# Stanford-NavLab/NavLab-DPE-SDR

Hardware: AMD Instinct MI355X
Metric: manifold gridpoints x SVs correlated/sec (higher is better)
Workload: dtype f32

## Files before the change

### navlab-dpe-sdr_amd/csrc/dpe_bcs.hip

```cpp
#include <type_traits>

#include "dpe_common.h"
#include "dpe_prep.h"
#include "dpe_chm_dev.h"

namespace dpe {

constexpr int kSub = 256;
constexpr int kNMomMax = 6;
typedef float f2 __attribute__((ext_vector_type(2)));

__device__ __forceinline__ f2 cmul(f2 a, f2 b)
{
    f2 t, r;
    asm("v_pk_mul_f32 %0, %1, %2 op_sel_hi:[0,1]" : "=v"(t) : "v"(a), "v"(b));
    asm("v_pk_fma_f32 %0, %1, %2, %3 op_sel:[1,1,0] op_sel_hi:[1,0,1] neg_lo:[1,0,0]" : "=v"(r) : "v"(a), "v"(b), "v"(t));
    return r;
}

__device__ __forceinline__ f2 wipe_seed(float f)
{
    f2 w = f2{__builtin_amdgcn_cosf(f), -__builtin_amdgcn_sinf(f)};
    asm volatile("s_nop 1" : "+v"(w));
    return w;
// ... 35 lines not shown
        const int n4 = S >> 2;
        for (int n = gtid; n < n4; n += gsz) {
            const int4 v = x4[n];
            sI += (short)(v.x & 0xFFFF) + (short)(v.y & 0xFFFF) + (short)(v.z & 0xFFFF) + (short)(v.w & 0xFFFF);
            sQ += (v.x >> 16) + (v.y >> 16) + (v.z >> 16) + (v.w >> 16);
        }
        for (int n = (n4 << 2) + gtid; n < S; n += gsz) {
            const int v = x[n];
            sI += (short)(v & 0xFFFF);
            sQ += v >> 16;
        }
    } else {
        for (int n = gtid; n < S; n += gsz) {
            const int v = x[n];
            sI += (short)(v & 0xFFFF);
            sQ += v >> 16;
        }
    }
    long long tI = sI, tQ = sQ;
#pragma unroll
    for (int off = 32; off > 0; off >>= 1) {
        tI += __shfl_xor(tI, off, 64);
        tQ += __shfl_xor(tQ, off, 64);
    }
    __shared__ long long sW[4][2];
    if ((threadIdx.x & 63) == 0) { sW[threadIdx.x >> 6][0] = tI; sW[threadIdx.x >> 6][1] = tQ; }
    __syncthreads();
    if (threadIdx.x < 2) {
        long long *o = sums + ((size_t)w * kSumSlots + blockIdx.x) * 2;
        o[threadIdx.x] = sW[0][threadIdx.x] + sW[1][threadIdx.x] + sW[2][threadIdx.x] + sW[3][threadIdx.x];
    }
}

__global__ __launch_bounds__(256) void bcs_sum_kernel(const int16_t *__restrict__ iq, long long winStride, int S,
                                                      long long *__restrict__ sums, uint4 *__restrict__ upDst,
                                                      const uint4 *__restrict__ upSrc, int upN16)
{
    const int nThreads = gridDim.x * gridDim.y * 256;
    for (int i = (blockIdx.y * gridDim.x + blockIdx.x) * 256 + threadIdx.x; i < upN16; i += nThreads) upDst[i] = upSrc[i];
    sum_body(iq, winStride, S, sums);
}

struct BcsParamBlock {
    BcsChanDev c[DPE_MAX_CHAN];
    const int *guard;
};
__device__ __forceinline__ bool rerun_not_wanted(const BcsParamBlock &pb)
{
    return pb.guard != nullptr && (__hip_atomic_load(pb.guard, __ATOMIC_RELAXED, __HIP_MEMORY_SCOPE_AGENT) & 8) == 0;
}

__device__ __forceinline__ void window_mean(const long long *__restrict__ sums, int w, int nSumBlk, int S, float &mRe, float &mIm)
{
    const int lane = threadIdx.x & 63;
    long long tI = 0, tQ = 0;
    if (lane < nSumBlk) {
        const longlong2 v = *reinterpret_cast<const longlong2 *>(sums + ((size_t)w * kSumSlots + lane) * 2);
        tI = v.x; tQ = v.y;
    }
#pragma unroll
    for (int off = 32; off > 0; off >>= 1) {
        tI += __shfl_xor(tI, off, 64);
        tQ += __shfl_xor(tQ, off, 64);
    }
    mRe = (float)((double)tI / (double)(float)S);
    mIm = (float)((double)tQ / (double)(float)S);
}

template <int LH, int kNMom, bool TABLE, bool FUSE, bool CO = false>
__global__ __launch_bounds__(256) void bcs_bank_kernel(BcsParamBlock pb, int inl, const int16_t *__restrict__ iq, long long winStride, int S,
                                                       int K, int nSub, int tilesPerBlock, int nBlk, int vecOK, int nSumBlk, int lagShift,
                                                       const BcsChanDev *__restrict__ chan,
                                                       const long long *__restrict__ sums,
                                                       const int8_t *__restrict__ chipTable,
                                                       const double *__restrict__ tT,
                                                       float2 *__restrict__ part, float2 *__restrict__ mom,
                                                       float2 *__restrict__ momRep, long long *__restrict__ sumSlots, ChmKArgs co)
{
    constexpr int NL = 2 * LH + 1;
    constexpr int NREP = kSub + 2 * LH;
    constexpr int NRR = 4 + 2 * LH;
    __shared__ float sChips[2048];
    __shared__ __align__(16) float sRep[4][NREP + 4];
    __shared__ float2 sAcc[4][NL];
    if (rerun_not_wanted(pb)) return;

    int blkX = blockIdx.x;
    if constexpr (CO) {
        static_assert(FUSE && !TABLE, "the co-block rides in the single-window form");
        if (blkX == 0) {
            if (blockIdx.y == 0 && blockIdx.z == 0) chm_k2(co);
            else if (blockIdx.y == 1 && blockIdx.z == 0) chm_k3(co);
            return;
        }
        blkX -= 1;
    }
    const int blk = blkX, k = blockIdx.y, w = blockIdx.z;
    const int tid = threadIdx.x, wave = tid >> 6, lane = tid & 63;
    (void)pb;
    const BcsChanDev ch = params_ptr(chan, inl)[w * K + k];
    for (int i = tid; i < 2048; i += 256) sChips[i] = (float)chipTable[(ch.prn - 1) * 1024 + (i >= kLCA ? i - kLCA : i) % kLCA];
    const bool fastIdx = (double)NREP * ch.codeStep < 1000.0;
    float mRe = 0.f, mIm = 0.f;
    if (!FUSE) window_mean(sums, w, nSumBlk, S, mRe, mIm);
    int sumI = 0, sumQ = 0;
    __shared__ int sSum[4][2];
    const int16_t *x = iq + (size_t)w * winStride * 2;
    float xp[4];
#pragma unroll
    for (int i = 0; i < 4; ++i) xp[i] = (float)(4 * lane + i) - 127.5f;
    __syncthreads();

    for (int side = 0; side < 2; ++side) {
        f2 acc[NL];
#pragma unroll
        for (int j = 0; j < NL; ++j) acc[j] = f2{0.f, 0.f};

        for (int t = 0; t < tilesPerBlock; ++t) {
            const int sub = (blk * tilesPerBlock + t) * 4 + wave;
            const int sub0 = sub * kSub;
            const int lo = sub0 - LH - lagShift, hi = sub0 + kSub - 1 + LH - lagShift;
            bool active = sub < nSub;
            if (active) {
                if (!ch.hasFlip) active = (side == 0);
                else if (lo >= 0 && hi < S) active = (side == 0) ? (lo < ch.idxNext) : (hi >= ch.idxNext);
            }
            const int n0 = sub0 + 4 * lane;
            float re[4], im[4];
            const bool countRaw = FUSE && k == 0 && side == 0 && sub < nSub;
            if (active || countRaw) {
                int rawv[4];
                if (vecOK && n0 + 3 < S) {
                    const int4 v = *reinterpret_cast<const int4 *>(x + 2 * (size_t)n0);
                    rawv[0] = v.x; rawv[1] = v.y; rawv[2] = v.z; rawv[3] = v.w;
                } else {
#pragma unroll
                    for (int i = 0; i < 4; ++i) rawv[i] = (n0 + i < S) ? *reinterpret_cast<const int *>(x + 2 * (size_t)(n0 + i)) : 0;
                }
#pragma unroll
                for (int i = 0; i < 4; ++i) {
                    re[i] = (float)(short)(rawv[i] & 0xFFFF);
                    im[i] = (float)(rawv[i] >> 16);
                    if (countRaw) { sumI += (short)(rawv[i] & 0xFFFF); sumQ += rawv[i] >> 16; }
                }
            }
            if (active) {
                if (fastIdx && lo >= 0 && hi < S) {
                    const int ci0 = (int)floor(code_phase<TABLE>(ch, tT, lo));
                    const int shift = (ci0 % kLCA) - ci0;
                    const bool straddle = ch.hasFlip && lo < ch.idxNext && hi >= ch.idxNext;
                    for (int e = lane; e < NREP; e += 64) {
                        const int m = lo + e;
                        const int ci = (int)floor(code_phase<TABLE>(ch, tT, m)) + shift;
                        float r = sChips[ci];
                        if (straddle) r = ((m >= ch.idxNext) == (side == 1)) ? r : 0.f;
                        sRep[wave][e] = r;
                    }
                } else {
                    for (int e = lane; e < NREP; e += 64) {
                        int m = lo + e;
                        if (m < 0) m += S; else if (m >= S) m -= S;
                        const double cph = code_phase<TABLE>(ch, tT, m);
                        const int ci = ((int)floor(cph)) % kLCA;
                        const int sd = ch.hasFlip ? (m >= ch.idxNext) : 0;
                        sRep[wave][e] = (sd == side) ? sChips[ci] : 0.f;
                    }
                }
            }
            f2 M[kNMom], Mq[FUSE ? kNMom : 1];
#pragma unroll
            for (int p = 0; p < kNMom; ++p) M[p] = f2{0.f, 0.f};
#pragma unroll
            for (int p = 0; p < (FUSE ? kNMom : 1); ++p) Mq[p] = f2{0.f, 0.f};
            if (active) {
                double ph = carr_phase<TABLE>(ch, tT, n0 < S ? n0 : S - 1);
                ph -= floor(ph);
                const float f = (float)ph;
                f2 wv = wipe_seed(f);
                const f2 meanv = f2{mRe, mIm}, rotv = f2{ch.rotRe, ch.rotIm};
                float rr[NRR];
#pragma unroll
                for (int q = 0; q < NRR / 4; ++q) {
                    const float4 v = *reinterpret_cast<const float4 *>(&sRep[wave][4 * lane + 4 * q]);
                    rr[4 * q] = v.x; rr[4 * q + 1] = v.y; rr[4 * q + 2] = v.z; rr[4 * q + 3] = v.w;
                }
#pragma unroll
                for (int i = 0; i < 4; ++i) {
                    const f2 wrot = wv;
                    wv = table_fix<TABLE>(wrot, ch, tT, n0, i, S);
                    const f2 bb = cmul(f2{re[i], im[i]}, wv);
#pragma unroll
                    for (int j = 0; j < NL; ++j) {
                        const float r = rr[i + 2 * LH - j];
                        acc[j] = __builtin_elementwise_fma(bb, f2{r, r}, acc[j]);
                    }
                    const float r0 = (n0 + i < S) ? rr[i + LH] : 0.f;
                    if (FUSE) {
                        f2 cp = bb * r0, cq = wv * r0;
#pragma unroll
                        for (int p = 0; p < kNMom; ++p) {
                            M[p] += cp; Mq[p] += cq;
                            cp *= xp[i]; cq *= xp[i];
                        }
                    } else {
                        f2 cp = (bb - cmul(meanv, wv)) * r0;
#pragma unroll
                        for (int p = 0; p < kNMom; ++p) {
                            M[p] += cp;
                            cp *= xp[i];
                        }
                    }
                    wv = cmul(wrot, rotv);
                }
            }
            if (sub < nSub && lagShift == 0) {
                const size_t mo = ((((size_t)w * K + k) * 2 + side) * nSub + sub) * kNMom;
                float2 *o = mom + mo;
                if (active) {
                    float mm[2 * kNMom];
#pragma unroll
                    for (int p = 0; p < kNMom; ++p) { mm[2 * p] = M[p].x; mm[2 * p + 1] = M[p].y; }
                    dpp_sum_lane63(mm);
                    if (lane == 63) {
#pragma unroll
                        for (int p = 0; p < kNMom; ++p) o[p] = make_float2(mm[2 * p], mm[2 * p + 1]);
                    }
                    if (FUSE) {
#pragma unroll
                        for (int p = 0; p < kNMom; ++p) { mm[2 * p] = Mq[p].x; mm[2 * p + 1] = Mq[p].y; }
                        dpp_sum_lane63(mm);
                        if (lane == 63) {
#pragma unroll
                            for (int p = 0; p < kNMom; ++p) momRep[mo + p] = make_float2(mm[2 * p], mm[2 * p + 1]);
                        }
                    }
                } else if (lane < kNMom) {
                    o[lane] = make_float2(0.f, 0.f);
                    if (FUSE) momRep[mo + lane] = make_float2(0.f, 0.f);
                }
            }
        }
        {
            float aa[2 * NL];
#pragma unroll
            for (int j = 0; j < NL; ++j) { aa[2 * j] = acc[j].x; aa[2 * j + 1] = acc[j].y; }
            dpp_sum_lane63(aa);
            if (lane == 63) {
#pragma unroll
                for (int j = 0; j < NL; ++j) sAcc[wave][j] = make_float2(aa[2 * j], aa[2 * j + 1]);
            }
        }
        if (FUSE && k == 0 && side == 0) {
#pragma unroll
            for (int off = 32; off > 0; off >>= 1) {
                sumI += __shfl_xor(sumI, off, 64);
                sumQ += __shfl_xor(sumQ, off, 64);
            }
            if (lane == 0) { sSum[wave][0] = sumI; sSum[wave][1] = sumQ; }
        }
        __syncthreads();
        if (FUSE && k == 0 && side == 0 && tid < 2)
            sumSlots[((size_t)w * kSumSlots + blk) * 2 + tid] =
                (long long)sSum[0][tid] + (long long)sSum[1][tid] + (long long)sSum[2][tid] + (long long)sSum[3][tid];
        for (int j = tid; j < NL; j += 256) {
            float2 s = sAcc[0][j];
            s.x += sAcc[1][j].x; s.y += sAcc[1][j].y;
            s.x += sAcc[2][j].x; s.y += sAcc[2][j].y;
            s.x += sAcc[3][j].x; s.y += sAcc[3][j].y;
            part[((((size_t)w * K + k) * nBlk + blk) * 2 + side) * NL + j] = s;
        }
        __syncthreads();
    }
}

constexpr int kB16Blocks = 4;
template <int LH, int kNMom, bool TABLE>
__global__ __launch_bounds__(256, (LH <= 4 && !TABLE) ? kB16Blocks : 3) void bcs_bank16_kernel(BcsParamBlock pb, int inl, const int16_t *__restrict__ iq, long long winStride,
                                                         int S, int K, int nW, int nSub, int tilesPerBlock, int nBlk, int vecOK, int nSumBlk,
                                                         const BcsChanDev *__restrict__ chan,
                                                         const long long *__restrict__ sums,
                                                         const int8_t *__restrict__ chipTable,
                                                         const double *__restrict__ tT,
                                                         float2 *__restrict__ part, float2 *__restrict__ mom)
{
    constexpr int NL = 2 * LH + 1;
    constexpr int kPass = 1024;
    constexpr int NREP = kPass + 2 * LH;
    constexpr int NRR = 16 + 2 * LH;
    static_assert((8 + 2 * LH) % 4 == 0 && LH <= 8, "a segment's replica window is read as float4s");
    __shared__ float sChips[2048];
#ifdef DPE_B16_PAD
    constexpr int kRepLen = ((NREP + 8 + 15) / 16) * 20;
#define DPE_PAD16(e) ((e) + 4 * ((e) >> 4))
#else
    constexpr int kRepLen = NREP + 8;
#define DPE_PAD16(e) (e)
#endif
    __shared__ __align__(16) float sRep[4][kRepLen];
    __shared__ float2 sAcc[4][NL];

    const int slot = blockIdx.x >> 3, k = slot % K, tg = (slot / K) * 8 + (blockIdx.x & 7);
    if (tg >= nBlk * nW) return;
    const int w = tg / nBlk, blk = tg - w * nBlk;
    const int tid = threadIdx.x, wave = tid >> 6, lane = tid & 63;
    (void)pb;
    const BcsChanDev ch = params_ptr(chan, inl)[w * K + k];
    for (int i = tid; i < 2048; i += 256) sChips[i] = (float)chipTable[(ch.prn - 1) * 1024 + (i >= kLCA ? i - kLCA : i) % kLCA];
    const bool fastIdx = (double)NREP * ch.codeStep < 1000.0;
    float mRe, mIm;
    window_mean(sums, w, nSumBlk, S, mRe, mIm);
    const f2 meanv = f2{mRe, mIm}, rotv = f2{ch.rotRe, ch.rotIm};
    const int16_t *x = iq + (size_t)w * winStride * 2;
    const int padLane = DPE_PAD16(lane);
    (void)padLane;
    const float xbase = (float)(16 * (lane & 15)) - 127.5f;
    __syncthreads();

    for (int side = 0; side < 2; ++side) {
        f2 acc[NL];
#pragma unroll
        for (int j = 0; j < NL; ++j) acc[j] = f2{0.f, 0.f};
        bool anyActive = false;

        for (int t = 0; t < tilesPerBlock; ++t) {
            const int pass = (blk * tilesPerBlock + t) * 4 + wave;
            const int c0 = pass * kPass;
            const int lo = c0 - LH, hi = c0 + kPass - 1 + LH;
            bool active = c0 < S;
            if (active) {
                if (!ch.hasFlip) active = (side == 0);
                else if (lo >= 0 && hi < S) active = (side == 0) ? (lo < ch.idxNext) : (hi >= ch.idxNext);
            }
            anyActive |= active;
            const int n0 = c0 + 16 * lane;
            if (active) {
                if (fastIdx && lo >= 0 && hi < S) {
                    const int ci0 = (int)code_phase<TABLE>(ch, tT, lo);
                    const int shift = (ci0 % kLCA) - ci0;
                    const bool straddle = ch.hasFlip && lo < ch.idxNext && hi >= ch.idxNext;
                    if (!straddle) {
                        static_assert(NREP >= 1024 && NREP < 1024 + 64, "sixteen full rounds of 64 entries and a partial one");
                        if constexpr (TABLE) {
                            for (int e = lane; e < NREP; e += 64) sRep[wave][DPE_PAD16(e)] = sChips[(int)code_phase<TABLE>(ch, tT, lo + e) + shift];
                        } else {
#pragma unroll
                        for (int e0 = 0; e0 < 1024; e0 += 512) {
                            float v[8];
#pragma unroll
                            for (int j = 0; j < 8; ++j) v[j] = sChips[(int)code_phase<TABLE>(ch, tT, lo + e0 + 64 * j + lane) + shift];
#pragma unroll
                            for (int j = 0; j < 8; ++j) sRep[wave][DPE_PAD16(e0 + 64 * j) + padLane] = v[j];
                        }
                        if (1024 + lane < NREP) sRep[wave][DPE_PAD16(1024) + padLane] = sChips[(int)code_phase<TABLE>(ch, tT, lo + 1024 + lane) + shift];
                        }
                    } else {
                        for (int e = lane; e < NREP; e += 64) {
                            const int m = lo + e;
                            const float r = sChips[(int)code_phase<TABLE>(ch, tT, m) + shift];
                            sRep[wave][DPE_PAD16(e)] = ((m >= ch.idxNext) == (side == 1)) ? r : 0.f;
                        }
                    }
                } else {
                    for (int e = lane; e < NREP; e += 64) {
                        int m = lo + e;
                        if (m < 0) m += S; else if (m >= S) m -= S;
                        const double cph = code_phase<TABLE>(ch, tT, m);
                        const int ci = ((int)floor(cph)) % kLCA;
                        const int sd = ch.hasFlip ? (m >= ch.idxNext) : 0;
                        sRep[wave][DPE_PAD16(e)] = (sd == side) ? sChips[ci] : 0.f;
                    }
                }
            }
            f2 M[kNMom];
#pragma unroll
            for (int p = 0; p < kNMom; ++p) M[p] = f2{0.f, 0.f};
            auto segments = [&](auto allInTag) {
                constexpr bool kAllIn = decltype(allInTag)::value;
#pragma unroll 1
                for (int seg = 0; seg < 2; ++seg) {
                    const int ns = n0 + 8 * seg;
                    int raw[8];
                    if (vecOK && (kAllIn || ns + 7 < S)) {
#pragma unroll
                        for (int q = 0; q < 2; ++q) {
                            const int4 v = *reinterpret_cast<const int4 *>(x + 2 * (size_t)(ns + 4 * q));
                            raw[4 * q] = v.x; raw[4 * q + 1] = v.y; raw[4 * q + 2] = v.z; raw[4 * q + 3] = v.w;
                        }
                    } else {
#pragma unroll
                        for (int i = 0; i < 8; ++i) raw[i] = (ns + i < S) ? *reinterpret_cast<const int *>(x + 2 * (size_t)(ns + i)) : 0;
                    }
                    float rr[8 + 2 * LH];
#pragma unroll
                    for (int q = 0; q < (8 + 2 * LH) / 4; ++q) {
                        const float4 v = *reinterpret_cast<const float4 *>(&sRep[wave][DPE_PAD16(16 * lane + 8 * seg + 4 * q)]);
                        rr[4 * q] = v.x; rr[4 * q + 1] = v.y; rr[4 * q + 2] = v.z; rr[4 * q + 3] = v.w;
                    }
                    double ph = carr_phase<TABLE>(ch, tT, (kAllIn || ns < S) ? ns : S - 1);
                    ph -= floor(ph);
                    f2 wv = wipe_seed((float)ph);
                    const bool inside = kAllIn || ns + 7 < S;
                    f2 m[kNMom];
#pragma unroll
                    for (int p = 0; p < kNMom; ++p) m[p] = f2{0.f, 0.f};
#pragma unroll
                    for (int i = 0; i < 8; ++i) {
                        const f2 rawv = f2{(float)(short)(raw[i] & 0xFFFF), (float)(raw[i] >> 16)};
                        const f2 wrot = wv;
                        wv = table_fix<TABLE>(wrot, ch, tT, ns, i, S);
                        const f2 bb = cmul(rawv, wv);
#pragma unroll
                        for (int j = 0; j < NL; ++j) {
                            const float r = rr[i + 2 * LH - j];
                            acc[j] = __builtin_elementwise_fma(bb, f2{r, r}, acc[j]);
                        }
                        const float r0 = (inside || ns + i < S) ? rr[i + LH] : 0.f;
                        const f2 cp = (bb - cmul(meanv, wv)) * r0;
                        const float d = (float)i - 3.5f;
                        float dp = 1.f;
                        m[0] += cp;
#pragma unroll
                        for (int p = 1; p < kNMom; ++p) {
                            dp *= d;
                            m[p] = __builtin_elementwise_fma(cp, f2{dp, dp}, m[p]);
                        }
                        wv = cmul(wrot, rotv);
                    }
                    const float xc = xbase + (float)(8 * seg) + 3.5f;
                    float xpow[kNMom];
                    xpow[0] = 1.f;
#pragma unroll
                    for (int e = 1; e < kNMom; ++e) xpow[e] = xpow[e - 1] * xc;
                    constexpr float bin[6][6] = {{1, 0, 0, 0, 0, 0}, {1, 1, 0, 0, 0, 0}, {1, 2, 1, 0, 0, 0}, {1, 3, 3, 1, 0, 0}, {1, 4, 6, 4, 1, 0}, {1, 5, 10, 10, 5, 1}};
#pragma unroll
                    for (int p = 0; p < kNMom; ++p) {
                        M[p] += m[p];
#pragma unroll
                        for (int q = 0; q < p; ++q) {
                            const float cf = bin[p][q] * xpow[p - q];
                            M[p] = __builtin_elementwise_fma(m[q], f2{cf, cf}, M[p]);
                        }
                    }
                }
            };
            if (active) {
                if (c0 + kPass <= S) segments(std::true_type{});
                else segments(std::false_type{});
            }
            {
                const int sub = pass * 4 + (lane >> 4);
                float2 *o = mom + ((((size_t)w * K + k) * 2 + side) * nSub + sub) * kNMom;
                if (active) {
                    float mm[2 * kNMom];
#pragma unroll
                    for (int p = 0; p < kNMom; ++p) { mm[2 * p] = M[p].x; mm[2 * p + 1] = M[p].y; }
                    dpp_sum_rows(mm);
                    if (sub < nSub && (lane & 15) == 15) {
#pragma unroll
                        for (int p = 0; p < kNMom; ++p) o[p] = make_float2(mm[2 * p], mm[2 * p + 1]);
                    }
                } else if (sub < nSub && (lane & 15) < kNMom) {
                    o[lane & 15] = make_float2(0.f, 0.f);
                }
            }
        }
        if (anyActive) {
            float aa[2 * NL];
#pragma unroll
            for (int j = 0; j < NL; ++j) { aa[2 * j] = acc[j].x; aa[2 * j + 1] = acc[j].y; }
            dpp_sum_lane63(aa);
            if (lane == 63) {
#pragma unroll
                for (int j = 0; j < NL; ++j) sAcc[wave][j] = make_float2(aa[2 * j], aa[2 * j + 1]);
            }
        } else if (lane < NL) {
            sAcc[wave][lane] = make_float2(0.f, 0.f);
        }
        __syncthreads();
        for (int j = tid; j < NL; j += 256) {
            float2 s = sAcc[0][j];
            s.x += sAcc[1][j].x; s.y += sAcc[1][j].y;
            s.x += sAcc[2][j].x; s.y += sAcc[2][j].y;
            s.x += sAcc[3][j].x; s.y += sAcc[3][j].y;
            part[((((size_t)w * K + k) * nBlk + blk) * 2 + side) * NL + j] = s;
        }
        __syncthreads();
    }
}

#undef DPE_PAD16

template <int kNMom, bool TABLE>
__global__ __launch_bounds__(256) void bcs_bank_wide_kernel(BcsParamBlock pb, int inl, const int16_t *__restrict__ iq, long long winStride, int S,
                                                            int K, int nSub, int tilesPerBlock, int nBlk, int vecOK, int nSumBlk, int lagShift,
                                                            const BcsChanDev *__restrict__ chan,
                                                            const long long *__restrict__ sums,
                                                            const int8_t *__restrict__ chipTable,
                                                            const double *__restrict__ tT,
                                                            float2 *__restrict__ part, float2 *__restrict__ mom)
{
    constexpr int LH = 32, NL = 2 * LH + 1;
    constexpr int NREP = kSub + LH + 1;
    constexpr int NB = kSub + 2 * LH;
    __shared__ float sChips[2048];
    __shared__ float sRep[4][NREP + 3];
    __shared__ float2 sB[4][NB];
    __shared__ float2 sAcc[4][NL];
    if (rerun_not_wanted(pb)) return;

    const int blk = blockIdx.x, k = blockIdx.y, w = blockIdx.z;
    const int tid = threadIdx.x, wave = tid >> 6, lane = tid & 63;
    (void)pb;
    const BcsChanDev ch = params_ptr(chan, inl)[w * K + k];
    for (int i = tid; i < 2048; i += 256) sChips[i] = (float)chipTable[(ch.prn - 1) * 1024 + (i >= kLCA ? i - kLCA : i) % kLCA];
    const bool fastIdx = (double)NREP * ch.codeStep < 1000.0;
    float mRe, mIm;
    window_mean(sums, w, nSumBlk, S, mRe, mIm);
    const int16_t *x = iq + (size_t)w * winStride * 2;
    float xp[4];
#pragma unroll
    for (int i = 0; i < 4; ++i) xp[i] = (float)(4 * lane + i) - 127.5f;
    __syncthreads();

    for (int side = 0; side < 2; ++side) {
        f2 acc0 = f2{0.f, 0.f};
        f2 D = f2{0.f, 0.f};
        for (int t = 0; t < tilesPerBlock; ++t) {
            const int sub = (blk * tilesPerBlock + t) * 4 + wave;
            const int sub0 = sub * kSub;
            const int lo = sub0 - 1 - lagShift, hi = sub0 + kSub - 1 + LH - lagShift;
            bool active = sub < nSub;
            if (active) {
                if (!ch.hasFlip) active = (side == 0);
                else if (lo >= 0 && hi < S) active = (side == 0) ? (lo < ch.idxNext) : (hi >= ch.idxNext);
            }
            f2 M[kNMom];
#pragma unroll
            for (int p = 0; p < kNMom; ++p) M[p] = f2{0.f, 0.f};
            if (active) {
                if (fastIdx && lo >= 0 && hi < S) {
                    const int ci0 = (int)floor(code_phase<TABLE>(ch, tT, lo));
                    const int shift = (ci0 % kLCA) - ci0;
                    const bool straddle = ch.hasFlip && lo < ch.idxNext && hi >= ch.idxNext;
                    for (int e = lane; e < NREP; e += 64) {
                        const int m = lo + e;
                        float r = sChips[(int)floor(code_phase<TABLE>(ch, tT, m)) + shift];
                        if (straddle) r = ((m >= ch.idxNext) == (side == 1)) ? r : 0.f;
                        sRep[wave][e] = r;
                    }
                } else {
                    for (int e = lane; e < NREP; e += 64) {
                        int m = lo + e;
                        if (m < 0) m += S; else if (m >= S) m -= S;
                        const int ci = ((int)floor(code_phase<TABLE>(ch, tT, m))) % kLCA;
                        const int sd = ch.hasFlip ? (m >= ch.idxNext) : 0;
                        sRep[wave][e] = (sd == side) ? sChips[ci] : 0.f;
                    }
                }
                const int n0 = sub0 + 4 * lane;
                float re[4], im[4];
                if (vecOK && n0 + 3 < S) {
                    const int4 v = *reinterpret_cast<const int4 *>(x + 2 * (size_t)n0);
                    re[0] = (float)(short)(v.x & 0xFFFF); im[0] = (float)(v.x >> 16);
                    re[1] = (float)(short)(v.y & 0xFFFF); im[1] = (float)(v.y >> 16);
                    re[2] = (float)(short)(v.z & 0xFFFF); im[2] = (float)(v.z >> 16);
                    re[3] = (float)(short)(v.w & 0xFFFF); im[3] = (float)(v.w >> 16);
                } else {
#pragma unroll
                    for (int i = 0; i < 4; ++i) {
                        int nn = n0 + i;
                        if (nn >= S) nn -= S;
                        const int v = *reinterpret_cast<const int *>(x + 2 * (size_t)nn);
                        re[i] = (float)(short)(v & 0xFFFF);
                        im[i] = (float)(v >> 16);
                    }
                }
                f2 bown[4], wown[4];
                {
                    int nn = n0 >= S ? n0 - S : n0;
                    double ph = carr_phase<TABLE>(ch, tT, nn);
                    ph -= floor(ph);
                    const float f = (float)ph;
                    f2 wv = wipe_seed(f);
                    const f2 rotv = f2{ch.rotRe, ch.rotIm};
                    int seedIdx = nn, steps = 0;
#pragma unroll
                    for (int i = 0; i < 4; ++i) {
                        if (n0 + i == S) {
                            double p2 = ch.ri - floor(ch.ri);
                            wv = wipe_seed((float)p2);
                            seedIdx = 0; steps = 0;
                        }
                        const f2 wrot = wv;
                        wv = table_fix<TABLE>(wrot, ch, tT, seedIdx, steps, S);
                        ++steps;
                        wown[i] = wv;
                        bown[i] = cmul(f2{re[i], im[i]}, wv);
                        sB[wave][LH + 4 * lane + i] = make_float2(bown[i].x, bown[i].y);
                        wv = cmul(wrot, rotv);
                    }
                }
                {
                    int nh = (lane < LH) ? (sub0 - LH + lane) : (sub0 + kSub + lane - LH);
                    const int e = (lane < LH) ? lane : (kSub + lane);
                    if (nh < 0) nh += S; else if (nh >= S) nh -= S;
                    const int v = *reinterpret_cast<const int *>(x + 2 * (size_t)nh);
                    const float hr = (float)(short)(v & 0xFFFF), hi2 = (float)(v >> 16);
                    double ph = carr_phase<TABLE>(ch, tT, nh);
                    ph -= floor(ph);
                    const float f = (float)ph;
                    const float wr = __builtin_amdgcn_cosf(f), wi = -__builtin_amdgcn_sinf(f);
                    sB[wave][e] = make_float2(hr * wr - hi2 * wi, hr * wi + hi2 * wr);
                }
#pragma unroll
                for (int i = 0; i < 4; ++i) {
                    const bool real = n0 + i < S;
                    const float rl = real ? sRep[wave][4 * lane + i + 1 + LH] : 0.f;
                    acc0 = __builtin_elementwise_fma(bown[i], f2{rl, rl}, acc0);
                    const float r0 = real ? sRep[wave][4 * lane + i + 1] : 0.f;
                    f2 cp = (bown[i] - cmul(f2{mRe, mIm}, wown[i])) * r0;
#pragma unroll
                    for (int p = 0; p < kNMom; ++p) {
                        M[p] += cp;
                        cp *= xp[i];
                    }
                }
#pragma unroll
                for (int i = 0; i < 4; ++i) {
                    const int e = 4 * lane + i;
                    const float J = (sub0 + e < S) ? (sRep[wave][e] - sRep[wave][e + 1]) : 0.f;
                    unsigned long long mask = __ballot(J != 0.f);
                    while (mask) {
                        const int src = __builtin_ctzll(mask);
                        mask &= mask - 1;
                        const float Jv = __builtin_bit_cast(float, __builtin_amdgcn_readlane(__builtin_bit_cast(int, J), src));
                        const float2 bv = sB[wave][4 * src + i + lane];
                        D = __builtin_elementwise_fma(f2{bv.x, bv.y}, f2{Jv, Jv}, D);
                    }
                }
            }
            if (sub < nSub && lagShift == 0) {
                float2 *o = mom + ((((size_t)w * K + k) * 2 + side) * nSub + sub) * kNMom;
                if (active) {
                    float mm[2 * kNMom];
#pragma unroll
                    for (int p = 0; p < kNMom; ++p) { mm[2 * p] = M[p].x; mm[2 * p + 1] = M[p].y; }
                    dpp_sum_lane63(mm);
                    if (lane == 63) {
#pragma unroll
                        for (int p = 0; p < kNMom; ++p) o[p] = make_float2(mm[2 * p], mm[2 * p + 1]);
                    }
                } else if (lane < kNMom) {
                    o[lane] = make_float2(0.f, 0.f);
                }
            }
        }
        {
            float aa[3] = {acc0.x, acc0.y, 0.f};
            dpp_sum_lane63(aa);
            if (lane == 63) sAcc[wave][0] = make_float2(aa[0], aa[1]);
            sAcc[wave][1 + lane] = make_float2(D.x, D.y);
        }
        __syncthreads();
        for (int j = tid; j < NL; j += 256) {
// ... 1070 lines not shown
```

Baseline: 2271 billion.

## Add fast replica path for edge and straddle passes, simplify chip phase math

Passes that straddle a flip or wrap around the window edge now use a shift-based, unrolled replica build instead of the slow double-precision floor/modulo path, using precomputed shifts for wrapped indices. The non-table interior path computes the code phase with a direct fma on a hoisted double base. The wave index is made uniform via readfirstlane, and the chip-table fill drops a modulo. This targets replica generation cost in the less common passes, at the risk of subtle indexing errors at wrap boundaries.

Measured after the change: 2281 billion, median of 6. Within noise of the previous version (+0.5%).

```diff
diff --git a/navlab-dpe-sdr_amd/csrc/dpe_bcs.hip b/navlab-dpe-sdr_amd/csrc/dpe_bcs.hip
--- a/navlab-dpe-sdr_amd/csrc/dpe_bcs.hip
+++ b/navlab-dpe-sdr_amd/csrc/dpe_bcs.hip
@@ -361,11 +361,25 @@
     const int slot = blockIdx.x >> 3, k = slot % K, tg = (slot / K) * 8 + (blockIdx.x & 7);
     if (tg >= nBlk * nW) return;
     const int w = tg / nBlk, blk = tg - w * nBlk;
-    const int tid = threadIdx.x, wave = tid >> 6, lane = tid & 63;
+    const int tid = threadIdx.x, wave = __builtin_amdgcn_readfirstlane(tid >> 6), lane = tid & 63;
     (void)pb;
     const BcsChanDev ch = params_ptr(chan, inl)[w * K + k];
-    for (int i = tid; i < 2048; i += 256) sChips[i] = (float)chipTable[(ch.prn - 1) * 1024 + (i >= kLCA ? i - kLCA : i) % kLCA];
+    {
+        const int8_t *ct = chipTable + (ch.prn - 1) * 1024;
+        for (int i = tid; i < 2048; i += 256) {
+            int c = i >= kLCA ? i - kLCA : i;
+            c = c >= kLCA ? c - kLCA : c;
+            sChips[i] = (float)ct[c];
+        }
+    }
     const bool fastIdx = (double)NREP * ch.codeStep < 1000.0;
+    const bool fastEdge = fastIdx && S >= NREP;
+    int shiftLo = 0, shiftHi = 0;
+    if (fastEdge) {
+        const int cl = (int)code_phase<TABLE>(ch, tT, S - LH), ch0 = (int)code_phase<TABLE>(ch, tT, 0);
+        shiftLo = (cl % kLCA) - cl;
+        shiftHi = (ch0 % kLCA) - ch0;
+    }
     float mRe, mIm;
     window_mean(sums, w, nSumBlk, S, mRe, mIm);
     const f2 meanv = f2{mRe, mIm}, rotv = f2{ch.rotRe, ch.rotIm};
@@ -393,32 +407,44 @@
             anyActive |= active;
             const int n0 = c0 + 16 * lane;
             if (active) {
-                if (fastIdx && lo >= 0 && hi < S) {
+                const bool interior = lo >= 0 && hi < S;
+                if (fastIdx && interior && !(ch.hasFlip && lo < ch.idxNext && hi >= ch.idxNext)) {
                     const int ci0 = (int)code_phase<TABLE>(ch, tT, lo);
                     const int shift = (ci0 % kLCA) - ci0;
-                    const bool straddle = ch.hasFlip && lo < ch.idxNext && hi >= ch.idxNext;
-                    if (!straddle) {
-                        static_assert(NREP >= 1024 && NREP < 1024 + 64, "sixteen full rounds of 64 entries and a partial one");
-                        if constexpr (TABLE) {
-                            for (int e = lane; e < NREP; e += 64) sRep[wave][DPE_PAD16(e)] = sChips[(int)code_phase<TABLE>(ch, tT, lo + e) + shift];
-                        } else {
+                    static_assert(NREP >= 1024 && NREP < 1024 + 64, "sixteen full rounds of 64 entries and a partial one");
+                    if constexpr (TABLE) {
+                        for (int e = lane; e < NREP; e += 64) sRep[wave][DPE_PAD16(e)] = sChips[(int)code_phase<TABLE>(ch, tT, lo + e) + shift];
+                    } else {
+                        const double dm = (double)(lo + lane);
 #pragma unroll
                         for (int e0 = 0; e0 < 1024; e0 += 512) {
                             float v[8];
 #pragma unroll
-                            for (int j = 0; j < 8; ++j) v[j] = sChips[(int)code_phase<TABLE>(ch, tT, lo + e0 + 64 * j + lane) + shift];
+                            for (int j = 0; j < 8; ++j) v[j] = sChips[(int)fma(dm + (double)(e0 + 64 * j), ch.codeStep, ch.rc) + shift];
 #pragma unroll
                             for (int j = 0; j < 8; ++j) sRep[wave][DPE_PAD16(e0 + 64 * j) + padLane] = v[j];
                         }
-                        if (1024 + lane < NREP) sRep[wave][DPE_PAD16(1024) + padLane] = sChips[(int)code_phase<TABLE>(ch, tT, lo + 1024 + lane) + shift];
-                        }
-                    } else {
-                        for (int e = lane; e < NREP; e += 64) {
-                            const int m = lo + e;
-                            const float r = sChips[(int)code_phase<TABLE>(ch, tT, m) + shift];
-                            sRep[wave][DPE_PAD16(e)] = ((m >= ch.idxNext) == (side == 1)) ? r : 0.f;
-                        }
-                    }
+                        if (1024 + lane < NREP) sRep[wave][DPE_PAD16(1024) + padLane] = sChips[(int)fma(dm + 1024.0, ch.codeStep, ch.rc) + shift];
+                    }
+                } else if (fastIdx && (interior || fastEdge)) {
+                    const int ci0 = (int)code_phase<TABLE>(ch, tT, lo < 0 ? 0 : lo);
+                    const int shift = (ci0 % kLCA) - ci0;
+                    auto entry = [&](int e) {
+                        int m = lo + e, sh = shift;
+                        if (m < 0) { m += S; sh = shiftLo; }
+                        else if (m >= S) { m -= S; sh = shiftHi; }
+                        const float r = sChips[(int)code_phase<TABLE>(ch, tT, m) + sh];
+                        return (!ch.hasFlip || (m >= ch.idxNext) == (side == 1)) ? r : 0.f;
+                    };
+#pragma unroll
+                    for (int e0 = 0; e0 < 1024; e0 += 512) {
+                        float v[8];
+#pragma unroll
+                        for (int j = 0; j < 8; ++j) v[j] = entry(e0 + 64 * j + lane);
+#pragma unroll
+                        for (int j = 0; j < 8; ++j) sRep[wave][DPE_PAD16(e0 + 64 * j) + padLane] = v[j];
+                    }
+                    if (1024 + lane < NREP) sRep[wave][DPE_PAD16(1024) + padLane] = entry(1024 + lane);
                 } else {
                     for (int e = lane; e < NREP; e += 64) {
                         int m = lo + e;
```
